# MiloszKrajewski/lz4net

Measured on AMD Instinct MI355X. Metric: uncompressed GB/s, batched 64KiB-block encode+decode: value = decode (known output size) per step over the whole resident batch; fast encode and LZ4HC encode of the same data in roofline_encode / roofline_hc, higher is better.
Workload: dtype u8

## Files before the change

lz4net_amd/csrc/lz4hip_decode_lane4.hpp:

```cpp
#pragma once
#include "lz4hip_common.hpp"
#include <type_traits>

#ifndef LZ4HIP_ITERATION_HOOK
#define LZ4HIP_ITERATION_HOOK(lane) ((void)0)
#endif
#ifndef LZ4HIP_STAT
#define LZ4HIP_STAT(slot, cond) ((void)0)
#endif
#ifdef LZ4HIP_SECTION_MARKERS
#define LZ4HIP_SECTION(name) asm volatile("; @@SECTION " name)
#else
#define LZ4HIP_SECTION(name) ((void)0)
#endif

namespace lz4hip {

#ifndef LZ4HIP_DEC4_FLUSH_RECS
#define LZ4HIP_DEC4_FLUSH_RECS 0
#endif
#ifndef LZ4HIP_DEC4_DUAL_STORE
#define LZ4HIP_DEC4_DUAL_STORE 2
#endif
constexpr unsigned lane4_lds_bytes(int ring_bytes) { return 64u * (unsigned)ring_bytes + 16u * 32u; }

struct NoNext {
    static constexpr bool kPersistent = false;
    LZ4HIP_DEVICE bool operator()(int, const uint8_t*&, int&, uint8_t*&, int&) const { return false; }
};

enum L4Kind { kK4None = 0, kK4Near = 1, kK4Far = 2, kK4Lit = 3, kK4Zero = 4 };
enum L4Flag { kF4Final = 1, kF4Err = 2, kF4Header = 4 };

template <bool KNOWN, int R, int P, int FU, int FS, int FE = 1, int IE = 1, int POL = 0, class NEXT = NoNext, int WAVES = 1>
LZ4HIP_DEVICE int lane4_decode_block(unsigned char* lds, int lane, bool active, const uint8_t* src, int iend,
                                     uint8_t* dst, int oend, NEXT next = NEXT(), int wave = 0)
{
    static_assert(WAVES == 1 || WAVES == 4, "one or four wavefronts per workgroup");
    constexpr uint32_t kRow = 256u * (uint32_t)WAVES;
    static_assert(R >= 128 && R % 16 == 0 && R <= 1008, "ring: a multiple of 16 bytes, 128 .. 1008");
    static_assert(P == 32 || P == 64, "input piece: 32 or 64 bytes");
    static_assert(FU == 64 || (FU == 128 && R >= 192), "flush unit: 64 bytes, or 128 with a ring of at least 192");
    static_assert(FS == 1 || FS == 2, "one or two flush store instructions per iteration");
    static_assert(FE == 1 || FE == 2, "the flush runs in every iteration or in every second one");
    static_assert(IE == 1 || (IE == 2 && FE == 2), "input requests in every iteration, or alternating with the flush");
    constexpr int RW = R / 4;
    constexpr bool RPOW2 = (RW & (RW - 1)) == 0;
    constexpr uint32_t kRingBytes = (uint32_t)RW * kRow;
    constexpr uint32_t kLdsBytes = lane4_lds_bytes(R) * (uint32_t)WAVES;
    constexpr bool LS = (POL & 16) != 0;
    constexpr int kDual = (POL & 32) ? 0 : (LZ4HIP_DEC4_DUAL_STORE);
    static_assert(!LS || P == 32, "sector input feeds 32-byte pieces");
    constexpr int SK = LS ? 64 : P;
    constexpr int NW = 4 + P / 4, NL = LS ? 4 : P / 16;
    constexpr int HPR = FU / 16, RECS_PER_STORE = 64 / HPR;
    constexpr int kFlushRecs = (LZ4HIP_DEC4_FLUSH_RECS) ? (LZ4HIP_DEC4_FLUSH_RECS) : FS * RECS_PER_STORE;
    constexpr bool kLineNoWrap = R % 64 == 0;
    constexpr int kNearMax = R - 20;
    unsigned char* const frec_base = lds + kRingBytes + (uint32_t)wave * 256u;
    auto frec = [&](int i) -> Aligned16* {
        if (kFlushRecs <= 16) return (Aligned16*)(frec_base + (uint32_t)i * 16u);
        return (Aligned16*)(frec_base + (uint32_t)(i >> 4) * kRow + (uint32_t)(i & 15) * 16u);
    };
    const uint32_t lane4 = (uint32_t)(wave * 64 + lane) << 2;

    auto ring_add = [](uint32_t a, uint32_t rows256) -> uint32_t {
        const uint32_t t = a + rows256;
        if (RPOW2) return t & (kRingBytes - 1u);
        const uint32_t u = t - kRingBytes;
        return u < t ? u : t;
    };
#define L4_RING(a) (*(uint32_t*)(lds + (a)))
#define L4_PHASE_SEL(p_) wv::alignbyte(0x07060504u, 0x03020100u, (uint32_t)(p_) & 3u)

    int skew = 0, in_total = 0;
    uint64_t src_al = 0;
    uint32_t out_limit = 0;
    int ip = 0;
    uint32_t W[NW];
    wv::u32x4 L[NL];
    int wb = -16;
    int lvalid = 0;
    int pend_a = 0, pend_b = 0;
    int op = 0, fl = 0;
    uint32_t oa = lane4;
    int kind = kK4None, rem = 0, off = 8;
    int gready = 0;
    int pv = 0, p_ll = 0, p_st = 0, p_ml = 0, p_off = 0, p_flags = 0, p_res = 0;
    uint32_t p_l0 = 0, p_l1 = 0, p_l2 = 0;
    int hdr = 0;
    uint32_t token = 0;
    int final_seen = 0, final_run = 0, result = 0, done = 0;
    int exhausted = 0;
    wv::u32x4 fa = { 0, 0, 0, 0 }, fb = { 0, 0, 0, 0 };
#if defined(LZ4HIP_DEC4_BALLAST_VALU) || defined(LZ4HIP_DEC4_BALLAST_LDS)
    uint32_t ballast = 0;
#endif
#pragma unroll
    for (int j = 0; j < NW; j++) W[j] = 0;
#pragma unroll
    for (int j = 0; j < NL; j++) L[j] = wv::u32x4{ 0, 0, 0, 0 };
    auto start_block = [&](bool act) {
        skew = (int)((uint64_t)src & (uint64_t)(SK - 1));
        src_al = (uint64_t)src - (uint64_t)skew;
        in_total = iend > 0 ? (int)(((int64_t)skew + iend + P - 1) & ~(int64_t)(P - 1)) : 0;
        out_limit = oend > kLastLiterals ? (uint32_t)(oend - kLastLiterals) : 0u;
        ip = 0; wb = -16 - P; lvalid = 0; pend_a = 0; pend_b = 0; op = 0; fl = 0; oa = lane4;
        kind = kK4None; rem = 0; off = 8; gready = 0;
        pv = 0; p_ll = 0; p_st = 0; p_ml = 0; p_off = 0; p_flags = 0; p_res = 0; hdr = 0; token = 0;
        final_seen = 0; final_run = 0; result = 0; done = 0;
        if (!act || (!KNOWN && iend == 0)) { done = 1; final_seen = 1; }
    };
    start_block(active);

#define L4_STORE2(OFF_, v_) do { const uint32_t w_ = (v_); wv::lds_store_drop<OFF_>(lds, kLdsBytes, oa, w_); wv::lds_store_drop<OFF_>(lds, kLdsBytes, ob_, w_); } while (0)
#define L4_APPEND(d0_, d1_, d2_, d3_, n_, FOUR_)                                                         \
    do {                                                                                                \
        const uint32_t sb_ = (uint32_t)op & 3u;                                                         \
        const uint32_t s_ = wv::alignbyte(0x08070605u, 0x04030201u, sb_ ^ 3u);                          \
        wv::lds_mskor(&L4_RING(oa), 0xFFFFFFFFu << (8u * sb_), wv::perm(d0_, 0u, s_));                  \
        if (kDual) {                                                                                    \
                                                    \
            const uint32_t ob_ = oa - kRingBytes;                                                       \
            const uint32_t w1_ = wv::perm(d1_, d0_, s_), w2_ = wv::perm(d2_, d1_, s_);                  \
            if (kDual == 2) {                                         \
                wv::lds_store2_rows_drop<1 * WAVES, 2 * WAVES>(lds, kLdsBytes, oa, w1_, w2_);           \
                wv::lds_store2_rows_drop<1 * WAVES, 2 * WAVES>(lds, kLdsBytes, ob_, w1_, w2_);          \
                if (FOUR_) {                                                                            \
                    const uint32_t w3_ = wv::perm(d3_, d2_, s_), w4_ = wv::perm(0u, d3_, s_);           \
                    wv::lds_store2_rows_drop<3 * WAVES, 4 * WAVES>(lds, kLdsBytes, oa, w3_, w4_);       \
                    wv::lds_store2_rows_drop<3 * WAVES, 4 * WAVES>(lds, kLdsBytes, ob_, w3_, w4_);      \
                } else {                                                                                \
                    L4_STORE2(3 * kRow, wv::perm(0u, d2_, s_));                                         \
                }                                                                                       \
            } else {                                                                                    \
                L4_STORE2(kRow, w1_);                                                                   \
                L4_STORE2(2 * kRow, w2_);                                                               \
                if (FOUR_) {                                                                            \
                    L4_STORE2(3 * kRow, wv::perm(d3_, d2_, s_));                                        \
                    L4_STORE2(4 * kRow, wv::perm(0u, d3_, s_));                                         \
                } else {                                                                                \
                    L4_STORE2(3 * kRow, wv::perm(0u, d2_, s_));                                         \
                }                                                                                       \
            }                                                                                           \
        } else {                                                                                        \
            const uint32_t a1_ = ring_add(oa, kRow), a2_ = ring_add(oa, 2 * kRow), a3_ = ring_add(oa, 3 * kRow); \
            L4_RING(a1_) = wv::perm(d1_, d0_, s_);                                                      \
            L4_RING(a2_) = wv::perm(d2_, d1_, s_);                                                      \
            if (FOUR_) {                                                                                \
                L4_RING(a3_) = wv::perm(d3_, d2_, s_);                                                  \
                L4_RING(ring_add(oa, 4 * kRow)) = wv::perm(0u, d3_, s_);                                \
            } else {                                                                                    \
                L4_RING(a3_) = wv::perm(0u, d2_, s_);                                                   \
            }                                                                                           \
        }                                                                                               \
        oa = ring_add(oa, (((sb_ + (uint32_t)(n_)) << 6) & 0x700u) * (uint32_t)WAVES);                  \
        op += (n_);                                                                                     \
    } while (0)

    auto iteration = [&](auto flush_tag, wv::u32x4& ldF, wv::u32x4& usF, int& ld_pend, int& us_pend) __attribute__((always_inline)) -> bool {
        constexpr bool FLUSH = decltype(flush_tag)::value;
        constexpr bool INPUT = IE == 1 || !FLUSH;
        constexpr int kVm = (FLUSH ? FS : 0) + 1 + (INPUT ? NL : 0);
        LZ4HIP_ITERATION_HOOK(lane);
        LZ4HIP_SECTION("T1a window refill");
        int d = ip + skew - wb;
        {
            const bool no_more = wb + 16 + P >= in_total;
            const bool cross = (d >= P) & ((lvalid != 0) | no_more);
            const wv::mask_t cm = wv::cond(d >= P) & (wv::cond(lvalid != 0) | wv::cond(no_more));
#pragma unroll
            for (int j = 0; j < 4; j++) W[j] = wv::sel(cm, W[P / 4 + j], W[j]);
            if constexpr (LS) {
                const bool hi_half = ((wb + 16 + P) & 32) != 0;
                const wv::mask_t hm = wv::cond(((wb + 16 + P) & 32) != 0);
#pragma unroll
                for (int j = 0; j < 2; j++) {
                    W[4 + 4 * j] = wv::sel(cm, wv::sel(hm, L[2 + j].x, L[j].x), W[4 + 4 * j]); W[5 + 4 * j] = wv::sel(cm, wv::sel(hm, L[2 + j].y, L[j].y), W[5 + 4 * j]);
                    W[6 + 4 * j] = wv::sel(cm, wv::sel(hm, L[2 + j].z, L[j].z), W[6 + 4 * j]); W[7 + 4 * j] = wv::sel(cm, wv::sel(hm, L[2 + j].w, L[j].w), W[7 + 4 * j]);
                }
                lvalid = (cross & hi_half) ? 0 : lvalid;
            } else {
#pragma unroll
                for (int j = 0; j < NL; j++) {
                    W[4 + 4 * j] = wv::sel(cm, L[j].x, W[4 + 4 * j]); W[5 + 4 * j] = wv::sel(cm, L[j].y, W[5 + 4 * j]);
                    W[6 + 4 * j] = wv::sel(cm, L[j].z, W[6 + 4 * j]); W[7 + 4 * j] = wv::sel(cm, L[j].w, W[7 + 4 * j]);
                }
                lvalid = cross ? 0 : lvalid;
            }
            wb += cross ? P : 0;
            d -= cross ? P : 0;
        }
        LZ4HIP_SECTION("T1b cursor view (select tree + rotation)");
        const bool staged16 = d < P;
        LZ4HIP_STAT(0, true); LZ4HIP_STAT(1, done == 0); LZ4HIP_STAT(2, (done == 0) & !staged16);
        uint32_t x0, x1, x2, x3;
        {
            const uint32_t k = (uint32_t)d >> 2;
            uint32_t t[NW];
#pragma unroll
            for (int j = 0; j < NW; j++) t[j] = W[j];
            int n = NW;
#pragma unroll
            for (int sh = P / 8; sh >= 1; sh >>= 1) {
                const wv::mask_t m = wv::cond((k & (uint32_t)sh) != 0u);
                n -= sh;
#pragma unroll
                for (int j = 0; j < NW; j++)
                    if (j < n) t[j] = wv::sel(m, t[j + sh], t[j]);
            }
            const uint32_t sx = L4_PHASE_SEL(d);
            x0 = wv::perm(t[1], t[0], sx); x1 = wv::perm(t[2], t[1], sx); x2 = wv::perm(t[3], t[2], sx); x3 = wv::perm(t[4], t[3], sx);
        }
        LZ4HIP_SECTION("T1c near-match source rows");
        uint32_t v0, v1, v2, v3;
        {
            const uint32_t offn = kind == kK4Near ? (uint32_t)off : 4u;
            const uint32_t back = (((offn + 3u - ((uint32_t)op & 3u)) << 6) & ~0xFFu) * (uint32_t)WAVES;
            uint32_t sa;
            if (RPOW2) sa = (oa - back) & (kRingBytes - 1u);
            else { const uint32_t t = oa - back, u = t + kRingBytes; sa = u < t ? u : t; }
            const uint32_t r0 = L4_RING(sa), r1 = L4_RING(ring_add(sa, kRow)), r2 = L4_RING(ring_add(sa, 2 * kRow)),
                           r3 = L4_RING(ring_add(sa, 3 * kRow)), r4 = L4_RING(ring_add(sa, 4 * kRow));
            const uint32_t sr = L4_PHASE_SEL((uint32_t)op - offn);
            v0 = wv::perm(r1, r0, sr); v1 = wv::perm(r2, r1, sr); v2 = wv::perm(r3, r2, sr); v3 = wv::perm(r4, r3, sr);
        }

        LZ4HIP_SECTION("T2 cooperative flush");
        if constexpr (FLUSH) {
            const bool need = (done == 0) & (op - fl >= FU);
            const uint64_t needy = wv::ballot(need);
            const int cnt_all = wv::popc64(needy);
            const bool go = cnt_all != 0;
            int cnt = 0;
            bool mine = false;
            if (go) {
                cnt = cnt_all < kFlushRecs ? cnt_all : kFlushRecs;
                const int frank = wv::rank_below(needy);
                mine = need & (frank < kFlushRecs);
                if (mine) {
                    const uint64_t dp = (uint64_t)dst;
                    *frec(frank) = Aligned16{ { ring_add(oa, kRingBytes - ((((uint32_t)(op - fl)) << 6) & ~0xFFu) * (uint32_t)WAVES), (uint32_t)fl, (uint32_t)dp, (uint32_t)(dp >> 32) } };
                }
                wv::mem_sync();
            }
            const int sub = lane % HPR;
#pragma unroll
            for (int base = 0; base < FS * RECS_PER_STORE; base += RECS_PER_STORE) {
                const int idx = base + lane / HPR;
                const bool act = idx < cnt;
                const wv::mask_t act_m = wv::cond(idx < cnt);
                uint64_t g = 0;
                uint32_t q0 = 0, q1 = 0, q2 = 0, q3 = 0;
                if (act) {
                    const Aligned16 r = *frec(idx);
                    g = ((uint64_t)r.w[2] | ((uint64_t)r.w[3] << 32)) + (uint64_t)(r.w[1] + 16u * (uint32_t)sub);
                    const uint32_t b0 = ring_add(r.w[0], 4u * kRow * (uint32_t)sub);
                    if (kLineNoWrap) { q0 = L4_RING(b0); q1 = L4_RING(b0 + kRow); q2 = L4_RING(b0 + 2 * kRow); q3 = L4_RING(b0 + 3 * kRow); }
                    else { q0 = L4_RING(b0); q1 = L4_RING(ring_add(b0, kRow)); q2 = L4_RING(ring_add(b0, 2 * kRow)); q3 = L4_RING(ring_add(b0, 3 * kRow)); }
                }
                wv::vm_store16_mask(act_m, g, q0, q1, q2, q3);
            }
            LZ4HIP_STAT(3, need); LZ4HIP_STAT(4, need & !mine);
            if (go) {
                wv::mem_sync();
                fl += mine ? FU : 0;
            }
        }
        LZ4HIP_SECTION("T3 chunk size");
        const bool room = op - fl <= R - 46;
        const bool near = kind == kK4Near, lit = kind == kK4Lit;
        const bool can = room & (rem > 0) & !((kind == kK4Far) & (gready == 0)) & !(lit & !staged16);
        const int stride = (near & (off < 16)) ? off : 16;
        int n = can ? (rem < stride ? rem : stride) : 0;
        n = ((kind == kK4Zero) & (n > 8)) ? 8 : n;
        LZ4HIP_STAT(5, (done == 0) & (rem > 0)); LZ4HIP_STAT(6, (done == 0) & (rem > 0) & (n == 0)); LZ4HIP_STAT(7, (done == 0) & (rem > 0) & !room);
        LZ4HIP_STAT(8, (done == 0) & (rem > 0) & (kind == kK4Far) & (gready == 0)); LZ4HIP_STAT(9, (done == 0) & (rem > n));
        const int rem_after = rem - n;
        const int op_end = op + rem;

        LZ4HIP_SECTION("T4 parse ahead");
        const bool may_parse = (pv == 0) & (final_seen == 0) & !(lit & (rem > 0)) & staged16;
        LZ4HIP_STAT(10, may_parse); LZ4HIP_STAT(11, (done == 0) & (pv != 0));
        if (may_parse) {
            const uint32_t tok = hdr ? token : (x0 & 255u);
            const uint32_t t4 = tok >> 4, b1 = (x0 >> 8) & 255u, mlc = tok & 15u;
            const bool e1 = (hdr == 0) & (t4 == 15u), e2 = mlc == 15u;
            const int ll = hdr ? 0 : (int)t4 + (e1 ? (int)b1 : 0);
            const bool in_win = (hdr != 0) | (t4 <= 11u);
            const int o = hdr ? 0 : 1 + (int)t4;
            uint32_t ot;
            {
                const uint32_t q = (uint32_t)o >> 2;
                const wv::mask_t m1 = wv::cond((q & 1u) != 0u), m2 = wv::cond((q & 2u) != 0u);
                const uint32_t lo = wv::sel(m2, wv::sel(m1, x3, x2), wv::sel(m1, x1, x0));
                const uint32_t hi = wv::sel(m2, x3, wv::sel(m1, x2, x1));
                ot = wv::alignbyte(hi, lo, (uint32_t)o & 3u);
            }
            const int vo = (int)(ot & 0xFFFFu);
            const uint32_t extb = (ot >> 16) & 255u;
            const int ml = (int)mlc + kMinMatch + (e2 ? (int)extb : 0);
            const int lit_end = op_end + ll;
            const int p_after = ip + o + 2;
            bool trap = (ip + 16 > iend) | (e1 & (b1 == 255u)) | (ip + 1 + (e1 ? 1 : 0) + ll > iend);
            trap |= in_win & ((e2 & (extb == 255u)) | (vo > lit_end) | ((uint32_t)lit_end + (uint32_t)ml > out_limit));
            if (KNOWN) trap |= (hdr == 0) & (lit_end > oend - 8);
            else       trap |= ((hdr == 0) & ((lit_end > oend - kMfLimit) | (ip + 1 + (e1 ? 1 : 0) + ll > iend - 8))) | (in_win & e2 & !(p_after < iend - (kLastLiterals + 1)));
            p_l0 = wv::alignbyte(x1, x0, 1); p_l1 = wv::alignbyte(x2, x1, 1); p_l2 = wv::alignbyte(x3, x2, 1);
            token = tok;
            p_ll = in_win ? ll : 0;
            p_st = in_win ? 0 : ll;
            p_ml = in_win ? ml : 0;
            p_off = vo;
            p_flags = in_win ? 0 : (int)kF4Header;
            const int ip_fast = in_win ? p_after + (e2 ? 1 : 0) : ip + 1 + (e1 ? 1 : 0);
            if (trap) {
                LZ4HIP_SECTION("T4x byte-wise parser (trap)");
                int err = 0, pos = ip;
                if (!hdr) {
                    const uint32_t tk = ip < iend ? src[ip] : 0u;
                    int l = (int)(tk >> 4);
                    pos = ip + 1;
                    if (l == 15) {
                        uint32_t b = 255;
                        if (KNOWN) { do { b = pos < iend ? src[pos] : 0u; pos++; l += (int)b; if (l > (1 << 30)) { err = -pos; l = 0; break; } } while (b == 255); }
                        else       { while (pos < iend && b == 255) { b = src[pos]; pos++; l += (int)b; l = l > (1 << 30) ? (1 << 30) : l; } }
                    }
                    token = tk;
                    const int le = (int)((int64_t)op_end + l > 0x7FFFFFFF ? 0x7FFFFFFF : op_end + l);
                    const bool last = KNOWN ? (le > oend - 8) : ((le > oend - kMfLimit) | (pos + l > iend - 8));
                    p_ll = 0; p_st = l; p_ml = 0; p_off = 8;
                    if (last) {
                        if (KNOWN) { if (err == 0 && (le != oend || pos + l > iend)) err = -pos; }
                        else       { if (le > oend || pos + l != iend) err = -pos; }
                        p_flags = kF4Final;
                        p_res = KNOWN ? pos + l : le;
                        final_seen = 1;
                    } else {
                        if (KNOWN && err == 0 && pos + l > iend) err = -pos;
                        p_flags = kF4Header;
                    }
                    ip = pos;
                } else {
                    int p = ip;
                    const int o_ = (int)((p < iend ? src[p] : 0u) | ((p + 1 < iend ? src[p + 1] : 0u) << 8));
                    p += 2;
                    int m = (int)(token & 15u);
                    if (m == 15) {
                        if (KNOWN) {
                            uint32_t b;
                            while ((b = (p < iend ? src[p] : 0u)) == 255) { m += 255; p++; if (m > (1 << 30)) { err = -p; break; } }
                            m += (int)b; p++;
                        } else {
                            while (p < iend - (kLastLiterals + 1)) { const uint32_t b = src[p]; p++; m += (int)b; m = m > (1 << 30) ? (1 << 30) : m; if (b != 255) break; }
                        }
                    }
                    m += kMinMatch;
                    if (err != 0) {}
                    else if (op_end - o_ < 0) err = -(ip + 2);
                    else if ((int64_t)op_end + m > (int64_t)oend - kLastLiterals) err = -p;
                    p_ll = 0; p_st = 0; p_ml = m; p_off = o_; p_flags = 0;
                    ip = p;
                    hdr = 0;
                }
                if (err != 0) { p_flags = kF4Err; p_res = err; }
                hdr = (p_flags & kF4Header) ? 1 : 0;
            } else {
                ip = ip_fast;
                hdr = in_win ? 0 : 1;
            }
            LZ4HIP_SECTION("T4 parse ahead");
            pv = 1;
        }

        LZ4HIP_SECTION("T5 far fetch");
        {
            const wv::mask_t m_rem0 = wv::cond(rem_after == 0);
            const wv::mask_t f_cont = wv::cond(kind == kK4Far) & ~m_rem0;
            const wv::mask_t f_first = m_rem0 & wv::cond(op - fl <= R - 46) & wv::cond(pv != 0) & wv::cond(p_ml != 0) & wv::cond(p_flags == 0) & wv::cond(p_off > kNearMax);
            const int f_pos = (int)wv::sel(f_cont, (uint32_t)(op + n - off), (uint32_t)(op_end + p_ll - p_off));
            const wv::mask_t f_want = f_cont | f_first;
            const wv::mask_t f_do = f_want & wv::cond(f_pos + 16 <= fl);
            wv::vm_load16_mask<POL & 3>(f_do, (uint64_t)dst + (uint64_t)(uint32_t)f_pos, ldF);
            gready = (int)wv::sel(f_do, 1u, 0u);
            LZ4HIP_STAT(15, gready != 0); LZ4HIP_STAT(16, wv::sel(f_want & ~f_do, 1u, 0u) != 0u);
        }

        LZ4HIP_SECTION("T6 input request");
        if constexpr (INPUT) {
            const int lpos = wb + 16 + P;
            const wv::mask_t req = wv::cond((done | lvalid | us_pend) == 0) & wv::cond(lpos < in_total);
            const uint64_t g = src_al + (uint64_t)(uint32_t)lpos;
            wv::vm_load16_mask_off<(POL >> 2) & 3, 0>(req, g, L[0]);
            wv::vm_load16_mask_off<(POL >> 2) & 3, 16>(req, g, L[1]);
            if constexpr (NL == 4) {
                wv::vm_load16_mask_off<(POL >> 2) & 3, 32>(req, g, L[2]);
                wv::vm_load16_mask_off<(POL >> 2) & 3, 48>(req, g, L[3]);
            }
            ld_pend = (int)wv::sel(req, 1u, 0u);
        } else {
            ld_pend = 0;
        }

        LZ4HIP_SECTION("B1 wait");
        wv::vm_wait_list<kVm>(usF, L);
        lvalid = us_pend ? 1 : lvalid;
        us_pend = 0;

#if defined(LZ4HIP_DEC4_BALLAST_VALU) || defined(LZ4HIP_DEC4_BALLAST_LDS)
#ifdef LZ4HIP_DEC4_BALLAST_VALU
#pragma unroll
        for (int bi = 0; bi < LZ4HIP_DEC4_BALLAST_VALU; bi++) asm volatile("v_add_u32 %0, %0, %1" : "+v"(ballast) : "v"(lane4));
#endif
#ifdef LZ4HIP_DEC4_BALLAST_LDS
#pragma unroll
        for (int bi = 0; bi < LZ4HIP_DEC4_BALLAST_LDS; bi++) wv::lds_store_drop<0>(lds, kLdsBytes, 0x80000000u + lane4, ballast);
#endif
#endif
        LZ4HIP_SECTION("B3 chunk append");
        {
            const bool far_src = kind == kK4Far;
            v0 = lit ? x0 : (far_src ? usF.x : v0);
            v1 = lit ? x1 : (far_src ? usF.y : v1);
            v2 = lit ? x2 : (far_src ? usF.z : v2);
            v3 = lit ? x3 : (far_src ? usF.w : v3);
            if ((kind == kK4Zero) & (n > 0)) {
                uint64_t acc = 0;
                for (int b = 0; b < n; b++) acc |= (uint64_t)dst[op + b] << (8 * b);
                v0 = (uint32_t)acc; v1 = (uint32_t)(acc >> 32);
            }
            ip += lit ? n : 0;
            L4_APPEND(v0, v1, v2, v3, n, true);
            rem = rem_after;
            off = (near & (off < 16) & (n > 0)) ? off * 2 : off;
            kind = rem == 0 ? (int)kK4None : kind;
        }

        LZ4HIP_SECTION("B4 promote + literal append");
        {
            const bool promote = (rem == 0) & (pv != 0) & room;
            LZ4HIP_STAT(12, promote); LZ4HIP_STAT(13, (done == 0) & (rem == 0) & (pv != 0) & !room); LZ4HIP_STAT(14, (done == 0) & (rem == 0) & (pv == 0));
            const bool perr = promote & ((p_flags & kF4Err) != 0);
            const bool pgo = promote & !perr;
            L4_APPEND(p_l0, p_l1, p_l2, 0u, pgo ? p_ll : 0, false);
            if (perr) {
                done = 1; final_seen = 1; final_run = 0; result = p_res;
            }
            if (pgo) {
                const bool streamed = p_st > 0;
                rem = streamed ? p_st : p_ml;
                off = streamed ? off : p_off;
                kind = streamed ? (int)kK4Lit : (p_ml == 0 ? (int)kK4None : (p_off == 0 ? (int)kK4Zero : (p_off <= kNearMax ? (int)kK4Near : (int)kK4Far)));
                final_run = (p_flags & kF4Final) ? 1 : final_run;
                result = (p_flags & kF4Final) ? p_res : result;
            }
            pv = promote ? 0 : pv;
        }

        LZ4HIP_SECTION("B5 end of block + loop");
        if (final_run && rem == 0 && !pv && !done) {
            uint32_t qa = ring_add(oa, kRingBytes - ((((uint32_t)(op - fl)) << 6) & ~0xFFu) * (uint32_t)WAVES);
            while (op - fl >= 4) { const uint32_t qd = L4_RING(qa); __builtin_memcpy(dst + fl, &qd, 4); fl += 4; qa = ring_add(qa, kRow); }
            if (fl < op) {
                const uint32_t qd = L4_RING(qa);
                for (int b = 0; fl + b < op; b++) dst[fl + b] = (uint8_t)(qd >> (8 * b));
            }
            done = 1;
        }
        return !wv::any(done == 0);
    };

    for (;;) {
        if (!std::remove_reference<NEXT>::type::kPersistent) {
            if (iteration(std::true_type{}, fa, fb, pend_a, pend_b)) break;
            if (iteration(std::integral_constant<bool, FE == 1>{}, fb, fa, pend_b, pend_a)) break;
        } else {
            (void)iteration(std::true_type{}, fa, fb, pend_a, pend_b);
            (void)iteration(std::integral_constant<bool, FE == 1>{}, fb, fa, pend_b, pend_a);
            const bool fin = (done != 0) & (exhausted == 0);
            if (wv::any(fin)) {
                if (fin) {
                    if (next(result, src, iend, dst, oend)) start_block(true);
                    else exhausted = 1;
                }
                if (!wv::any(exhausted == 0)) break;
            }
        }
    }
    return result;
#undef L4_RING
#undef L4_PHASE_SEL
#undef L4_APPEND
#undef L4_STORE2
}

__global__ void __launch_bounds__(256) count_selected_kernel(Batch b, int filter, unsigned* count)
{
    unsigned mine = 0;
    for (int64_t blk = (int64_t)blockIdx.x * 256 + threadIdx.x; blk < b.n_blocks; blk += (int64_t)gridDim.x * 256)
        mine += block_selected(filter, batch_src_len(b, blk), batch_dst_cap(b, blk)) ? 1u : 0u;
    const unsigned total = wv::scan_add(mine);
    if ((threadIdx.x & 63u) == 63u && total) atomicAdd(count, total);
}
LZ4HIP_DEVICE bool lane4_gate_open(const unsigned* gate, int gate_mode, unsigned threshold)
{
    if (gate_mode == 0) return true;
    const unsigned c = wv::uniform(*gate);
    return gate_mode == 1 ? c >= threshold : c < threshold;
}

__global__ void __launch_bounds__(64) lds_drop_probe_kernel(unsigned* errors, int rounds)
{
    constexpr uint32_t kBytes = lane4_lds_bytes(192), kRing = 64u * 192u, kWords = kBytes / 4u;
    LZ4HIP_STATIC_LDS(lds, kBytes);
    uint32_t* const s = (uint32_t*)lds;
    const uint32_t lane = threadIdx.x, tag = 0x9E3779B9u * (blockIdx.x + 1u);
    for (uint32_t i = lane; i < kWords; i += 64u) s[i] = tag ^ i;
    wv::block_sync();
    for (int r = 0; r < rounds; r++) {
        const uint32_t junk = 0xDEAD0000u | (uint32_t)r;
        const uint32_t last = kRing - 256u + lane * 4u;
        const uint32_t own = tag ^ (last >> 2);
        wv::lds_store2_rows_drop<0, 3>(lds, kBytes, last, own, junk);
        wv::lds_store2_rows_drop<3, 4>(lds, kBytes, last, junk, junk);
        wv::lds_store_drop<1024>(lds, kBytes, last, junk);
        wv::lds_store_drop<768>(lds, kBytes, kBytes - 256u + lane * 4u, junk);
        const uint32_t neg = lane * 4u - kRing;
        wv::lds_store2_rows_drop<1, 2>(lds, kBytes, neg, junk, junk);
        wv::lds_store2_rows_drop<3, 4>(lds, kBytes, neg + 2048u, junk, junk);
        wv::lds_store_drop<768>(lds, kBytes, neg, junk);
        wv::lds_store2_rows_drop<0, 48>(lds, kBytes, neg, junk, tag ^ lane);
        wv::mem_sync();
#if defined(__HIP_DEVICE_COMPILE__)
        __builtin_amdgcn_s_sleep(8);
#endif
    }
    wv::block_sync();
    unsigned bad = 0;
// ... 77 lines not shown
```

lz4net_amd/csrc/lz4hip_wave.hpp:

```cpp
#pragma once
#include <hip/hip_runtime.h>
#include <stdint.h>

#define LZ4HIP_WAVE_API 1
#define LZ4HIP_DEVICE __device__ __forceinline__
#define LZ4HIP_DYN_LDS(name) extern __shared__ __attribute__((aligned(16))) unsigned char name[]
#define LZ4HIP_STATIC_LDS(name, bytes) __shared__ __attribute__((aligned(16))) unsigned char name[bytes]
#define LZ4HIP_KEEP(x) asm volatile("" : "+v"(x))

namespace wv {

constexpr int kWave = 64;

LZ4HIP_DEVICE int lane() { return (int)(threadIdx.x & 63u); }
LZ4HIP_DEVICE int wave_in_block() { return __builtin_amdgcn_readfirstlane((int)(threadIdx.x >> 6)); }

LZ4HIP_DEVICE uint32_t uniform(uint32_t v) { return (uint32_t)__builtin_amdgcn_readfirstlane((int)v); }
LZ4HIP_DEVICE int32_t uniform(int32_t v) { return __builtin_amdgcn_readfirstlane(v); }
LZ4HIP_DEVICE uint64_t uniform(uint64_t v)
{
    uint32_t lo = uniform((uint32_t)v), hi = uniform((uint32_t)(v >> 32));
    return ((uint64_t)hi << 32) | lo;
}
LZ4HIP_DEVICE int64_t uniform(int64_t v) { return (int64_t)uniform((uint64_t)v); }
// ... 67 lines not shown
    *(u32x4_unaligned*)p = v;
}
LZ4HIP_DEVICE void load16(const void* p, uint32_t& a, uint32_t& b, uint32_t& c, uint32_t& d)
{
    const u32x4_unaligned v = *(const u32x4_unaligned*)p;
    a = v.x; b = v.y; c = v.z; d = v.w;
}

typedef uint32_t u32x4 __attribute__((ext_vector_type(4)));
template <int POLICY = 0>
LZ4HIP_DEVICE void vm_load16_pred(bool pred, uint64_t addr, u32x4& v)
{
    const uint64_t m = __builtin_amdgcn_ballot_w64(pred);
    uint64_t saved;
#define LZ4HIP_VM_LOAD(MODS)                                                                                                      \
    asm volatile("s_and_saveexec_b64 %[sv], %[m]\n\tglobal_load_dwordx4 %[d], %[a], off" MODS "\n\ts_mov_b64 exec, %[sv]"       \
                 : [d] "+v"(v), [sv] "=&s"(saved) : [a] "v"(addr), [m] "s"(m) : "memory")
    if (POLICY == 1) LZ4HIP_VM_LOAD(" nt");
    else if (POLICY == 2) LZ4HIP_VM_LOAD(" sc1");
    else if (POLICY == 3) LZ4HIP_VM_LOAD(" sc0 sc1");
    else LZ4HIP_VM_LOAD("");
#undef LZ4HIP_VM_LOAD
}
LZ4HIP_DEVICE void vm_store16_pred(bool pred, uint64_t addr, uint32_t a, uint32_t b, uint32_t c, uint32_t d)
{
    const uint64_t m = __builtin_amdgcn_ballot_w64(pred);
    uint64_t saved;
    const u32x4 v = { a, b, c, d };
    asm volatile("s_and_saveexec_b64 %[sv], %[m]\n\tglobal_store_dwordx4 %[a], %[d], off\n\ts_mov_b64 exec, %[sv]"
                 : [sv] "=&s"(saved) : [a] "v"(addr), [d] "v"(v), [m] "s"(m) : "memory");
}
template <int N>
LZ4HIP_DEVICE void vm_wait(u32x4& a, u32x4& b)
{
    static_assert(N >= 0 && N < 64, "vmcnt is a 6-bit counter");
    asm volatile("s_waitcnt vmcnt(%[n])" : "+v"(a), "+v"(b) : [n] "n"(N) : "memory");
}

template <int N, int M>
LZ4HIP_DEVICE void vm_wait_list(u32x4& a, u32x4 (&l)[M])
{
    static_assert(N >= 0 && N < 64, "vmcnt is a 6-bit counter");
    asm volatile("s_waitcnt vmcnt(%[n])" : "+v"(a) : [n] "n"(N) : "memory");
#pragma unroll
    for (int j = 0; j < M; j++) asm volatile("" : "+v"(l[j]));
}

struct mask_t { uint64_t v; };
LZ4HIP_DEVICE mask_t cond(bool p) { return mask_t{ __builtin_amdgcn_ballot_w64(p) }; }
LZ4HIP_DEVICE mask_t operator&(mask_t a, mask_t b) { return mask_t{ a.v & b.v }; }
LZ4HIP_DEVICE mask_t operator|(mask_t a, mask_t b) { return mask_t{ a.v | b.v }; }
LZ4HIP_DEVICE mask_t operator~(mask_t a) { return mask_t{ ~a.v }; }
LZ4HIP_DEVICE bool any(mask_t m) { return m.v != 0ull; }
LZ4HIP_DEVICE uint32_t sel(mask_t m, uint32_t a, uint32_t b)
{
    uint32_t r;
    asm("v_cndmask_b32_e64 %0, %1, %2, %3" : "=v"(r) : "v"(b), "v"(a), "s"(m.v));
    return r;
}
template <int POLICY = 0>
LZ4HIP_DEVICE void vm_load16_mask(mask_t mk, uint64_t addr, u32x4& v)
{
    const uint64_t m = mk.v;
    uint64_t saved;
#define LZ4HIP_VM_LOAD(MODS)                                                                                                      \
    asm volatile("s_and_saveexec_b64 %[sv], %[m]\n\tglobal_load_dwordx4 %[d], %[a], off" MODS "\n\ts_mov_b64 exec, %[sv]"       \
                 : [d] "+v"(v), [sv] "=&s"(saved) : [a] "v"(addr), [m] "s"(m) : "memory")
    if (POLICY == 1) LZ4HIP_VM_LOAD(" nt");
    else if (POLICY == 2) LZ4HIP_VM_LOAD(" sc1");
    else if (POLICY == 3) LZ4HIP_VM_LOAD(" sc0 sc1");
    else LZ4HIP_VM_LOAD("");
#undef LZ4HIP_VM_LOAD
}
template <int POLICY, int OFF>
LZ4HIP_DEVICE void vm_load16_mask_off(mask_t mk, uint64_t addr, u32x4& v)
{
    static_assert(OFF >= 0 && OFF < 4096, "global_load offset field");
    const uint64_t m = mk.v;
    uint64_t saved;
#define LZ4HIP_VM_LOAD(MODS)                                                                                                                      \
    asm volatile("s_and_saveexec_b64 %[sv], %[m]\n\tglobal_load_dwordx4 %[d], %[a], off offset:%[o]" MODS "\n\ts_mov_b64 exec, %[sv]"       \
                 : [d] "+v"(v), [sv] "=&s"(saved) : [a] "v"(addr), [m] "s"(m), [o] "n"(OFF) : "memory")
    if (POLICY == 1) LZ4HIP_VM_LOAD(" nt");
    else if (POLICY == 2) LZ4HIP_VM_LOAD(" sc1");
    else if (POLICY == 3) LZ4HIP_VM_LOAD(" sc0 sc1");
    else LZ4HIP_VM_LOAD("");
#undef LZ4HIP_VM_LOAD
}
LZ4HIP_DEVICE void vm_store16_mask(mask_t mk, uint64_t addr, uint32_t a, uint32_t b, uint32_t c, uint32_t d)
{
    const uint64_t m = mk.v;
    uint64_t saved;
    const u32x4 v = { a, b, c, d };
    asm volatile("s_and_saveexec_b64 %[sv], %[m]\n\tglobal_store_dwordx4 %[a], %[d], off\n\ts_mov_b64 exec, %[sv]"
                 : [sv] "=&s"(saved) : [a] "v"(addr), [d] "v"(v), [m] "s"(m) : "memory");
}

LZ4HIP_DEVICE void lds_mskor(uint32_t* p, uint32_t mask, uint32_t data)
{
    asm volatile("ds_mskor_b32 %[a], %[m], %[d]" : : [a] "v"((uint32_t)(uintptr_t)(__attribute__((address_space(3))) uint32_t*)p), [m] "v"(mask), [d] "v"(data) : "memory");
}

template <int OFF>
LZ4HIP_DEVICE void lds_store_drop(unsigned char* lds, uint32_t lds_bytes, uint32_t a, uint32_t v)
{
    (void)lds_bytes;
// ... 23 lines not shown
```

Measured before the change: 1025.

## Keep per-lane decoder state flags as wave-wide scalar masks

Replaces the per-lane integer state flags (kind, lvalid, pending, pv, hdr, final/done/exhausted, parse flags) in the lane4 decoder with 64-bit wave masks held in scalar registers. Per-lane booleans are recovered with inverse_ballot when needed. The intent is to cut VGPR pressure and VALU compare/select work by doing flag logic with SALU mask operations, and to skip the zero-match and end-of-block paths wave-wide when no lane needs them. It adds SGPR pressure and inverse-ballot conversions, and it risks subtle state bugs in the persistent restart path.

```diff
diff --git a/lz4net_amd/csrc/lz4hip_decode_lane4.hpp b/lz4net_amd/csrc/lz4hip_decode_lane4.hpp
--- a/lz4net_amd/csrc/lz4hip_decode_lane4.hpp
+++ b/lz4net_amd/csrc/lz4hip_decode_lane4.hpp
@@ -14,6 +14,14 @@
 #define LZ4HIP_SECTION(name) ((void)0)
 #endif
 
+#ifndef LZ4HIP_WAVE_MASK_STATE
+namespace wv {
+inline mask_t mask_none() { return cond(false); }
+inline uint64_t ballot(mask_t m) { return ballot(m.v); }
+inline bool lane_of(mask_t m) { return m.v; }
+}
+#endif
+
 namespace lz4hip {
 
 #ifndef LZ4HIP_DEC4_FLUSH_RECS
@@ -28,9 +36,6 @@
     static constexpr bool kPersistent = false;
     LZ4HIP_DEVICE bool operator()(int, const uint8_t*&, int&, uint8_t*&, int&) const { return false; }
 };
-
-enum L4Kind { kK4None = 0, kK4Near = 1, kK4Far = 2, kK4Lit = 3, kK4Zero = 4 };
-enum L4Flag { kF4Final = 1, kF4Err = 2, kF4Header = 4 };
 
 template <bool KNOWN, int R, int P, int FU, int FS, int FE = 1, int IE = 1, int POL = 0, class NEXT = NoNext, int WAVES = 1>
 LZ4HIP_DEVICE int lane4_decode_block(unsigned char* lds, int lane, bool active, const uint8_t* src, int iend,
@@ -80,18 +85,22 @@
     uint32_t W[NW];
     wv::u32x4 L[NL];
     int wb = -16;
-    int lvalid = 0;
-    int pend_a = 0, pend_b = 0;
     int op = 0, fl = 0;
     uint32_t oa = lane4;
-    int kind = kK4None, rem = 0, off = 8;
-    int gready = 0;
-    int pv = 0, p_ll = 0, p_st = 0, p_ml = 0, p_off = 0, p_flags = 0, p_res = 0;
+    int rem = 0, off = 8;
+    int p_ll = 0, p_st = 0, p_ml = 0, p_off = 0, p_res = 0;
     uint32_t p_l0 = 0, p_l1 = 0, p_l2 = 0;
-    int hdr = 0;
     uint32_t token = 0;
-    int final_seen = 0, final_run = 0, result = 0, done = 0;
-    int exhausted = 0;
+    int result = 0;
+    wv::mask_t m_lvalid = wv::mask_none();
+    wv::mask_t m_pend_a = wv::mask_none(), m_pend_b = wv::mask_none();
+    wv::mask_t k_near = wv::mask_none(), k_far = wv::mask_none(), k_lit = wv::mask_none(), k_zero = wv::mask_none();
+    wv::mask_t m_gready = wv::mask_none();
+    wv::mask_t m_pv = wv::mask_none();
+    wv::mask_t pf_final = wv::mask_none(), pf_err = wv::mask_none();
+    wv::mask_t m_hdr = wv::mask_none();
+    wv::mask_t m_final_seen = wv::mask_none(), m_final_run = wv::mask_none(), m_done = wv::mask_none();
+    wv::mask_t m_exhausted = wv::mask_none();
     wv::u32x4 fa = { 0, 0, 0, 0 }, fb = { 0, 0, 0, 0 };
 #if defined(LZ4HIP_DEC4_BALLAST_VALU) || defined(LZ4HIP_DEC4_BALLAST_LDS)
     uint32_t ballast = 0;
@@ -100,18 +109,30 @@
     for (int j = 0; j < NW; j++) W[j] = 0;
 #pragma unroll
     for (int j = 0; j < NL; j++) L[j] = wv::u32x4{ 0, 0, 0, 0 };
-    auto start_block = [&](bool act) {
+    auto start_block = [&]() {
         skew = (int)((uint64_t)src & (uint64_t)(SK - 1));
         src_al = (uint64_t)src - (uint64_t)skew;
         in_total = iend > 0 ? (int)(((int64_t)skew + iend + P - 1) & ~(int64_t)(P - 1)) : 0;
         out_limit = oend > kLastLiterals ? (uint32_t)(oend - kLastLiterals) : 0u;
-        ip = 0; wb = -16 - P; lvalid = 0; pend_a = 0; pend_b = 0; op = 0; fl = 0; oa = lane4;
-        kind = kK4None; rem = 0; off = 8; gready = 0;
-        pv = 0; p_ll = 0; p_st = 0; p_ml = 0; p_off = 0; p_flags = 0; p_res = 0; hdr = 0; token = 0;
-        final_seen = 0; final_run = 0; result = 0; done = 0;
-        if (!act || (!KNOWN && iend == 0)) { done = 1; final_seen = 1; }
+        ip = 0; wb = -16 - P; op = 0; fl = 0; oa = lane4;
+        rem = 0; off = 8;
+        p_ll = 0; p_st = 0; p_ml = 0; p_off = 0; p_res = 0; token = 0;
+        result = 0;
     };
-    start_block(active);
+    auto start_masks = [&](wv::mask_t started, wv::mask_t dead) {
+        const wv::mask_t keep = ~started;
+        m_lvalid = m_lvalid & keep; m_pend_a = m_pend_a & keep; m_pend_b = m_pend_b & keep;
+        k_near = k_near & keep; k_far = k_far & keep; k_lit = k_lit & keep; k_zero = k_zero & keep; m_gready = m_gready & keep;
+        m_pv = m_pv & keep; pf_final = pf_final & keep; pf_err = pf_err & keep; m_hdr = m_hdr & keep;
+        m_final_run = m_final_run & keep;
+        m_final_seen = (m_final_seen & keep) | dead;
+        m_done = (m_done & keep) | dead;
+    };
+    start_block();
+    {
+        const bool dead = !active || (!KNOWN && iend == 0);
+        start_masks(~wv::mask_none(), wv::cond(dead));
+    }
 
 #define L4_STORE2(OFF_, v_) do { const uint32_t w_ = (v_); wv::lds_store_drop<OFF_>(lds, kLdsBytes, oa, w_); wv::lds_store_drop<OFF_>(lds, kLdsBytes, ob_, w_); } while (0)
 #define L4_APPEND(d0_, d1_, d2_, d3_, n_, FOUR_)                                                         \
@@ -158,7 +179,7 @@
         op += (n_);                                                                                     \
     } while (0)
 
-    auto iteration = [&](auto flush_tag, wv::u32x4& ldF, wv::u32x4& usF, int& ld_pend, int& us_pend) __attribute__((always_inline)) -> bool {
+    auto iteration = [&](auto flush_tag, wv::u32x4& ldF, wv::u32x4& usF, wv::mask_t& ld_pend, wv::mask_t& us_pend) __attribute__((always_inline)) -> bool {
         constexpr bool FLUSH = decltype(flush_tag)::value;
         constexpr bool INPUT = IE == 1 || !FLUSH;
         constexpr int kVm = (FLUSH ? FS : 0) + 1 + (INPUT ? NL : 0);
@@ -167,33 +188,32 @@
         int d = ip + skew - wb;
         {
             const bool no_more = wb + 16 + P >= in_total;
-            const bool cross = (d >= P) & ((lvalid != 0) | no_more);
-            const wv::mask_t cm = wv::cond(d >= P) & (wv::cond(lvalid != 0) | wv::cond(no_more));
+            const wv::mask_t cm = wv::cond(d >= P) & (m_lvalid | wv::cond(no_more));
+            const bool cross = wv::lane_of(cm);
 #pragma unroll
             for (int j = 0; j < 4; j++) W[j] = wv::sel(cm, W[P / 4 + j], W[j]);
             if constexpr (LS) {
-                const bool hi_half = ((wb + 16 + P) & 32) != 0;
                 const wv::mask_t hm = wv::cond(((wb + 16 + P) & 32) != 0);
 #pragma unroll
                 for (int j = 0; j < 2; j++) {
                     W[4 + 4 * j] = wv::sel(cm, wv::sel(hm, L[2 + j].x, L[j].x), W[4 + 4 * j]); W[5 + 4 * j] = wv::sel(cm, wv::sel(hm, L[2 + j].y, L[j].y), W[5 + 4 * j]);
                     W[6 + 4 * j] = wv::sel(cm, wv::sel(hm, L[2 + j].z, L[j].z), W[6 + 4 * j]); W[7 + 4 * j] = wv::sel(cm, wv::sel(hm, L[2 + j].w, L[j].w), W[7 + 4 * j]);
                 }
-                lvalid = (cross & hi_half) ? 0 : lvalid;
+                m_lvalid = m_lvalid & ~(cm & hm);
             } else {
 #pragma unroll
                 for (int j = 0; j < NL; j++) {
                     W[4 + 4 * j] = wv::sel(cm, L[j].x, W[4 + 4 * j]); W[5 + 4 * j] = wv::sel(cm, L[j].y, W[5 + 4 * j]);
                     W[6 + 4 * j] = wv::sel(cm, L[j].z, W[6 + 4 * j]); W[7 + 4 * j] = wv::sel(cm, L[j].w, W[7 + 4 * j]);
                 }
-                lvalid = cross ? 0 : lvalid;
+                m_lvalid = m_lvalid & ~cm;
             }
             wb += cross ? P : 0;
             d -= cross ? P : 0;
         }
         LZ4HIP_SECTION("T1b cursor view (select tree + rotation)");
-        const bool staged16 = d < P;
-        LZ4HIP_STAT(0, true); LZ4HIP_STAT(1, done == 0); LZ4HIP_STAT(2, (done == 0) & !staged16);
+        const wv::mask_t m_staged = wv::cond(d < P);
+        LZ4HIP_STAT(0, true); LZ4HIP_STAT(1, wv::lane_of(~m_done)); LZ4HIP_STAT(2, wv::lane_of(~m_done & ~m_staged));
         uint32_t x0, x1, x2, x3;
         {
             const uint32_t k = (uint32_t)d >> 2;
@@ -215,7 +235,7 @@
         LZ4HIP_SECTION("T1c near-match source rows");
         uint32_t v0, v1, v2, v3;
         {
-            const uint32_t offn = kind == kK4Near ? (uint32_t)off : 4u;
+            const uint32_t offn = wv::lane_of(k_near) ? (uint32_t)off : 4u;
             const uint32_t back = (((offn + 3u - ((uint32_t)op & 3u)) << 6) & ~0xFFu) * (uint32_t)WAVES;
             uint32_t sa;
             if (RPOW2) sa = (oa - back) & (kRingBytes - 1u);
@@ -228,8 +248,9 @@
 
         LZ4HIP_SECTION("T2 cooperative flush");
         if constexpr (FLUSH) {
-            const bool need = (done == 0) & (op - fl >= FU);
-            const uint64_t needy = wv::ballot(need);
+            const wv::mask_t need_m = ~m_done & wv::cond(op - fl >= FU);
+            const bool need = wv::lane_of(need_m);
+            const uint64_t needy = wv::ballot(need_m);
             const int cnt_all = wv::popc64(needy);
             const bool go = cnt_all != 0;
             int cnt = 0;
@@ -268,26 +289,31 @@
             }
         }
         LZ4HIP_SECTION("T3 chunk size");
-        const bool room = op - fl <= R - 46;
-        const bool near = kind == kK4Near, lit = kind == kK4Lit;
-        const bool can = room & (rem > 0) & !((kind == kK4Far) & (gready == 0)) & !(lit & !staged16);
-        const int stride = (near & (off < 16)) ? off : 16;
-        int n = can ? (rem < stride ? rem : stride) : 0;
-        n = ((kind == kK4Zero) & (n > 8)) ? 8 : n;
-        LZ4HIP_STAT(5, (done == 0) & (rem > 0)); LZ4HIP_STAT(6, (done == 0) & (rem > 0) & (n == 0)); LZ4HIP_STAT(7, (done == 0) & (rem > 0) & !room);
-        LZ4HIP_STAT(8, (done == 0) & (rem > 0) & (kind == kK4Far) & (gready == 0)); LZ4HIP_STAT(9, (done == 0) & (rem > n));
+        const wv::mask_t m_room = wv::cond(op - fl <= R - 46);
+        const wv::mask_t m_rem = wv::cond(rem > 0);
+        const wv::mask_t m_can = m_room & m_rem & ~(k_far & ~m_gready) & ~(k_lit & ~m_staged);
+        const wv::mask_t m_short = k_near & wv::cond(off < 16);
+        const bool lit = wv::lane_of(k_lit);
+        const int stride = wv::lane_of(m_short) ? off : 16;
+        int n = wv::lane_of(m_can) ? (rem < stride ? rem : stride) : 0;
+        if (wv::any(k_zero)) n = (wv::lane_of(k_zero) & (n > 8)) ? 8 : n;
+        LZ4HIP_STAT(5, wv::lane_of(~m_done & m_rem)); LZ4HIP_STAT(6, wv::lane_of(~m_done & m_rem) & (n == 0)); LZ4HIP_STAT(7, wv::lane_of(~m_done & m_rem & ~m_room));
+        LZ4HIP_STAT(8, wv::lane_of(~m_done & m_rem & k_far & ~m_gready)); LZ4HIP_STAT(9, wv::lane_of(~m_done) & (rem > n));
         const int rem_after = rem - n;
         const int op_end = op + rem;
 
         LZ4HIP_SECTION("T4 parse ahead");
-        const bool may_parse = (pv == 0) & (final_seen == 0) & !(lit & (rem > 0)) & staged16;
-        LZ4HIP_STAT(10, may_parse); LZ4HIP_STAT(11, (done == 0) & (pv != 0));
+        const wv::mask_t m_parse = ~m_pv & ~m_final_seen & ~(k_lit & m_rem) & m_staged;
+        const bool may_parse = wv::lane_of(m_parse);
+        LZ4HIP_STAT(10, may_parse); LZ4HIP_STAT(11, wv::lane_of(~m_done & m_pv));
+        bool n_hdr = false, n_final = false, n_err = false;
         if (may_parse) {
+            const bool hdr = wv::lane_of(m_hdr);
             const uint32_t tok = hdr ? token : (x0 & 255u);
             const uint32_t t4 = tok >> 4, b1 = (x0 >> 8) & 255u, mlc = tok & 15u;
-            const bool e1 = (hdr == 0) & (t4 == 15u), e2 = mlc == 15u;
+            const bool e1 = !hdr & (t4 == 15u), e2 = mlc == 15u;
             const int ll = hdr ? 0 : (int)t4 + (e1 ? (int)b1 : 0);
-            const bool in_win = (hdr != 0) | (t4 <= 11u);
+            const bool in_win = hdr | (t4 <= 11u);
             const int o = hdr ? 0 : 1 + (int)t4;
             uint32_t ot;
             {
@@ -304,15 +330,14 @@
             const int p_after = ip + o + 2;
             bool trap = (ip + 16 > iend) | (e1 & (b1 == 255u)) | (ip + 1 + (e1 ? 1 : 0) + ll > iend);
             trap |= in_win & ((e2 & (extb == 255u)) | (vo > lit_end) | ((uint32_t)lit_end + (uint32_t)ml > out_limit));
-            if (KNOWN) trap |= (hdr == 0) & (lit_end > oend - 8);
-            else       trap |= ((hdr == 0) & ((lit_end > oend - kMfLimit) | (ip + 1 + (e1 ? 1 : 0) + ll > iend - 8))) | (in_win & e2 & !(p_after < iend - (kLastLiterals + 1)));
+            if (KNOWN) trap |= !hdr & (lit_end > oend - 8);
+            else       trap |= (!hdr & ((lit_end > oend - kMfLimit) | (ip + 1 + (e1 ? 1 : 0) + ll > iend - 8))) | (in_win & e2 & !(p_after < iend - (kLastLiterals + 1)));
             p_l0 = wv::alignbyte(x1, x0, 1); p_l1 = wv::alignbyte(x2, x1, 1); p_l2 = wv::alignbyte(x3, x2, 1);
             token = tok;
             p_ll = in_win ? ll : 0;
             p_st = in_win ? 0 : ll;
             p_ml = in_win ? ml : 0;
             p_off = vo;
-            p_flags = in_win ? 0 : (int)kF4Header;
             const int ip_fast = in_win ? p_after + (e2 ? 1 : 0) : ip + 1 + (e1 ? 1 : 0);
             if (trap) {
                 LZ4HIP_SECTION("T4x byte-wise parser (trap)");
@@ -333,12 +358,11 @@
                     if (last) {
                         if (KNOWN) { if (err == 0 && (le != oend || pos + l > iend)) err = -pos; }
                         else       { if (le > oend || pos + l != iend) err = -pos; }
-                        p_flags = kF4Final;
+                        n_final = true;
                         p_res = KNOWN ? pos + l : le;
-                        final_seen = 1;
                     } else {
                         if (KNOWN && err == 0 && pos + l > iend) err = -pos;
-                        p_flags = kF4Header;
+                        n_hdr = true;
                     }
                     ip = pos;
                 } else {
@@ -359,37 +383,43 @@
                     if (err != 0) {}
                     else if (op_end - o_ < 0) err = -(ip + 2);
                     else if ((int64_t)op_end + m > (int64_t)oend - kLastLiterals) err = -p;
-                    p_ll = 0; p_st = 0; p_ml = m; p_off = o_; p_flags = 0;
+                    p_ll = 0; p_st = 0; p_ml = m; p_off = o_;
                     ip = p;
-                    hdr = 0;
                 }
-                if (err != 0) { p_flags = kF4Err; p_res = err; }
-                hdr = (p_flags & kF4Header) ? 1 : 0;
+                if (err != 0) { n_err = true; n_hdr = false; p_res = err; }
             } else {
                 ip = ip_fast;
-                hdr = in_win ? 0 : 1;
+                n_hdr = !in_win;
             }
             LZ4HIP_SECTION("T4 parse ahead");
-            pv = 1;
+        }
+        {
+            const wv::mask_t c_hdr = wv::cond(n_hdr), c_final = wv::cond(n_final), c_err = wv::cond(n_err);
+            m_hdr = (m_hdr & ~m_parse) | c_hdr;
+            pf_final = (pf_final & ~m_parse) | (c_final & ~c_err);
+            pf_err = (pf_err & ~m_parse) | c_err;
+            m_final_seen = m_final_seen | c_final;
+            m_pv = m_pv | m_parse;
         }
 
         LZ4HIP_SECTION("T5 far fetch");
+        const wv::mask_t m_rem0 = wv::cond(rem_after == 0);
+        const wv::mask_t m_pmatch = wv::cond(p_ml != 0), m_pfar = wv::cond(p_off > kNearMax);
         {
-            const wv::mask_t m_rem0 = wv::cond(rem_after == 0);
-            const wv::mask_t f_cont = wv::cond(kind == kK4Far) & ~m_rem0;
-            const wv::mask_t f_first = m_rem0 & wv::cond(op - fl <= R - 46) & wv::cond(pv != 0) & wv::cond(p_ml != 0) & wv::cond(p_flags == 0) & wv::cond(p_off > kNearMax);
+            const wv::mask_t f_cont = k_far & ~m_rem0;
+            const wv::mask_t f_first = m_rem0 & m_room & m_pv & m_pmatch & ~(pf_final | pf_err | m_hdr) & m_pfar;
             const int f_pos = (int)wv::sel(f_cont, (uint32_t)(op + n - off), (uint32_t)(op_end + p_ll - p_off));
             const wv::mask_t f_want = f_cont | f_first;
             const wv::mask_t f_do = f_want & wv::cond(f_pos + 16 <= fl);
             wv::vm_load16_mask<POL & 3>(f_do, (uint64_t)dst + (uint64_t)(uint32_t)f_pos, ldF);
-            gready = (int)wv::sel(f_do, 1u, 0u);
-            LZ4HIP_STAT(15, gready != 0); LZ4HIP_STAT(16, wv::sel(f_want & ~f_do, 1u, 0u) != 0u);
+            m_gready = f_do;
+            LZ4HIP_STAT(15, wv::lane_of(m_gready)); LZ4HIP_STAT(16, wv::lane_of(f_want & ~f_do));
         }
 
         LZ4HIP_SECTION("T6 input request");
         if constexpr (INPUT) {
             const int lpos = wb + 16 + P;
-            const wv::mask_t req = wv::cond((done | lvalid | us_pend) == 0) & wv::cond(lpos < in_total);
+            const wv::mask_t req = ~(m_done | m_lvalid | us_pend) & wv::cond(lpos < in_total);
             const uint64_t g = src_al + (uint64_t)(uint32_t)lpos;
             wv::vm_load16_mask_off<(POL >> 2) & 3, 0>(req, g, L[0]);
             wv::vm_load16_mask_off<(POL >> 2) & 3, 16>(req, g, L[1]);
@@ -397,15 +427,15 @@
                 wv::vm_load16_mask_off<(POL >> 2) & 3, 32>(req, g, L[2]);
                 wv::vm_load16_mask_off<(POL >> 2) & 3, 48>(req, g, L[3]);
             }
-            ld_pend = (int)wv::sel(req, 1u, 0u);
+            ld_pend = req;
         } else {
-            ld_pend = 0;
+            ld_pend = wv::mask_none();
         }
 
         LZ4HIP_SECTION("B1 wait");
         wv::vm_wait_list<kVm>(usF, L);
-        lvalid = us_pend ? 1 : lvalid;
-        us_pend = 0;
+        m_lvalid = m_lvalid | us_pend;
+        us_pend = wv::mask_none();
 
 #if defined(LZ4HIP_DEC4_BALLAST_VALU) || defined(LZ4HIP_DEC4_BALLAST_LDS)
 #ifdef LZ4HIP_DEC4_BALLAST_VALU
@@ -419,12 +449,12 @@
 #endif
         LZ4HIP_SECTION("B3 chunk append");
         {
-            const bool far_src = kind == kK4Far;
+            const bool far_src = wv::lane_of(k_far);
             v0 = lit ? x0 : (far_src ? usF.x : v0);
             v1 = lit ? x1 : (far_src ? usF.y : v1);
             v2 = lit ? x2 : (far_src ? usF.z : v2);
             v3 = lit ? x3 : (far_src ? usF.w : v3);
-            if ((kind == kK4Zero) & (n > 0)) {
+            if (wv::any(k_zero) && (wv::lane_of(k_zero) & (n > 0))) {
                 uint64_t acc = 0;
                 for (int b = 0; b < n; b++) acc |= (uint64_t)dst[op + b] << (8 * b);
                 v0 = (uint32_t)acc; v1 = (uint32_t)(acc >> 32);
@@ -432,58 +462,69 @@
             ip += lit ? n : 0;
             L4_APPEND(v0, v1, v2, v3, n, true);
             rem = rem_after;
-            off = (near & (off < 16) & (n > 0)) ? off * 2 : off;
-            kind = rem == 0 ? (int)kK4None : kind;
+            off = wv::lane_of(m_short & m_can) ? off * 2 : off;
+            { const wv::mask_t keep = ~m_rem0; k_near = k_near & keep; k_far = k_far & keep; k_lit = k_lit & keep; k_zero = k_zero & keep; }
         }
 
         LZ4HIP_SECTION("B4 promote + literal append");
         {
-            const bool promote = (rem == 0) & (pv != 0) & room;
-            LZ4HIP_STAT(12, promote); LZ4HIP_STAT(13, (done == 0) & (rem == 0) & (pv != 0) & !room); LZ4HIP_STAT(14, (done == 0) & (rem == 0) & (pv == 0));
-            const bool perr = promote & ((p_flags & kF4Err) != 0);
-            const bool pgo = promote & !perr;
+            const wv::mask_t m_promote = m_rem0 & m_pv & m_room;
+            LZ4HIP_STAT(12, wv::lane_of(m_promote)); LZ4HIP_STAT(13, wv::lane_of(~m_done & m_rem0 & m_pv & ~m_room)); LZ4HIP_STAT(14, wv::lane_of(~m_done & m_rem0 & ~m_pv));
+            const wv::mask_t m_perr = m_promote & pf_err;
+            const wv::mask_t m_pgo = m_promote & ~pf_err;
+            const bool pgo = wv::lane_of(m_pgo);
             L4_APPEND(p_l0, p_l1, p_l2, 0u, pgo ? p_ll : 0, false);
-            if (perr) {
-                done = 1; final_seen = 1; final_run = 0; result = p_res;
-            }
-            if (pgo) {
-                const bool streamed = p_st > 0;
-                rem = streamed ? p_st : p_ml;
-                off = streamed ? off : p_off;
-                kind = streamed ? (int)kK4Lit : (p_ml == 0 ? (int)kK4None : (p_off == 0 ? (int)kK4Zero : (p_off <= kNearMax ? (int)kK4Near : (int)kK4Far)));
-                final_run = (p_flags & kF4Final) ? 1 : final_run;
-                result = (p_flags & kF4Final) ? p_res : result;
-            }
-            pv = promote ? 0 : pv;
+            const wv::mask_t m_streamed = m_pgo & wv::cond(p_st > 0);
+            const wv::mask_t m_copy = m_pgo & ~m_streamed & m_pmatch;
+            const wv::mask_t m_zero = m_copy & wv::cond(p_off == 0);
+            rem = pgo ? (wv::lane_of(m_streamed) ? p_st : p_ml) : rem;
+            off = wv::lane_of(m_pgo & ~m_streamed) ? p_off : off;
+            k_lit = k_lit | m_streamed;
+            k_zero = k_zero | m_zero;
+            k_far = k_far | (m_copy & m_pfar);
+            k_near = k_near | (m_copy & ~m_pfar & ~m_zero);
+            result = wv::lane_of(m_perr | (m_pgo & pf_final)) ? p_res : result;
+            m_final_run = (m_final_run & ~m_perr) | (m_pgo & pf_final);
+            m_done = m_done | m_perr;
+            m_final_seen = m_final_seen | m_perr;
+            m_pv = m_pv & ~m_promote;
         }
 
         LZ4HIP_SECTION("B5 end of block + loop");
-        if (final_run && rem == 0 && !pv && !done) {
-            uint32_t qa = ring_add(oa, kRingBytes - ((((uint32_t)(op - fl)) << 6) & ~0xFFu) * (uint32_t)WAVES);
-            while (op - fl >= 4) { const uint32_t qd = L4_RING(qa); __builtin_memcpy(dst + fl, &qd, 4); fl += 4; qa = ring_add(qa, kRow); }
-            if (fl < op) {
-                const uint32_t qd = L4_RING(qa);
-                for (int b = 0; fl + b < op; b++) dst[fl + b] = (uint8_t)(qd >> (8 * b));
-            }
-            done = 1;
-        }
-        return !wv::any(done == 0);
+        const wv::mask_t m_ending = m_final_run & ~m_pv & ~m_done;
+        if (wv::any(m_ending)) {
+            const wv::mask_t m_end = m_ending & wv::cond(rem == 0);
+            if (wv::lane_of(m_end)) {
+                uint32_t qa = ring_add(oa, kRingBytes - ((((uint32_t)(op - fl)) << 6) & ~0xFFu) * (uint32_t)WAVES);
+                while (op - fl >= 4) { const uint32_t qd = L4_RING(qa); __builtin_memcpy(dst + fl, &qd, 4); fl += 4; qa = ring_add(qa, kRow); }
+                if (fl < op) {
+                    const uint32_t qd = L4_RING(qa);
+                    for (int b = 0; fl + b < op; b++) dst[fl + b] = (uint8_t)(qd >> (8 * b));
+                }
+            }
+            m_done = m_done | m_end;
+        }
+        return !wv::any(~m_done);
     };
 
     for (;;) {
         if (!std::remove_reference<NEXT>::type::kPersistent) {
-            if (iteration(std::true_type{}, fa, fb, pend_a, pend_b)) break;
-            if (iteration(std::integral_constant<bool, FE == 1>{}, fb, fa, pend_b, pend_a)) break;
+            if (iteration(std::true_type{}, fa, fb, m_pend_a, m_pend_b)) break;
+            if (iteration(std::integral_constant<bool, FE == 1>{}, fb, fa, m_pend_b, m_pend_a)) break;
         } else {
-            (void)iteration(std::true_type{}, fa, fb, pend_a, pend_b);
-            (void)iteration(std::integral_constant<bool, FE == 1>{}, fb, fa, pend_b, pend_a);
-            const bool fin = (done != 0) & (exhausted == 0);
-            if (wv::any(fin)) {
-                if (fin) {
-                    if (next(result, src, iend, dst, oend)) start_block(true);
-                    else exhausted = 1;
+            (void)iteration(std::true_type{}, fa, fb, m_pend_a, m_pend_b);
+            (void)iteration(std::integral_constant<bool, FE == 1>{}, fb, fa, m_pend_b, m_pend_a);
+            const wv::mask_t m_fin = m_done & ~m_exhausted;
+            if (wv::any(m_fin)) {
+                bool got = false;
+                if (wv::lane_of(m_fin)) {
+                    got = next(result, src, iend, dst, oend);
+                    if (got) start_block();
                 }
-                if (!wv::any(exhausted == 0)) break;
+                const wv::mask_t m_started = wv::cond(got);
+                start_masks(m_started, m_started & wv::cond(!KNOWN && iend == 0));
+                m_exhausted = m_exhausted | (m_fin & ~m_started);
+                if (!wv::any(~m_exhausted)) break;
             }
         }
     }
diff --git a/lz4net_amd/csrc/lz4hip_wave.hpp b/lz4net_amd/csrc/lz4hip_wave.hpp
--- a/lz4net_amd/csrc/lz4hip_wave.hpp
+++ b/lz4net_amd/csrc/lz4hip_wave.hpp
@@ -143,6 +143,10 @@
 LZ4HIP_DEVICE mask_t operator|(mask_t a, mask_t b) { return mask_t{ a.v | b.v }; }
 LZ4HIP_DEVICE mask_t operator~(mask_t a) { return mask_t{ ~a.v }; }
 LZ4HIP_DEVICE bool any(mask_t m) { return m.v != 0ull; }
+#define LZ4HIP_WAVE_MASK_STATE 1
+LZ4HIP_DEVICE mask_t mask_none() { return mask_t{ 0ull }; }
+LZ4HIP_DEVICE uint64_t ballot(mask_t m) { return m.v; }
+LZ4HIP_DEVICE bool lane_of(mask_t m) { return __builtin_amdgcn_inverse_ballot_w64(m.v); }
 LZ4HIP_DEVICE uint32_t sel(mask_t m, uint32_t a, uint32_t b)
 {
     uint32_t r;
```

New measurement: 1077, median of 6. 5.1% higher.
